# hustvl/4DGaussians

Hardware: NVIDIA H100
Metric: render FPS @300k gauss 1352x1014 (fused deform+rasterize forward); train-step ms in `train_step` (higher is better)
Workload: dtype f32

## Files before the change

### 4dgaussians_b200/csrc/g4d_api.cu

```cuda
#include <cstdio>
#include <cstdlib>
#include <atomic>
#include <cstring>
#include <mutex>
#include <string>
#include <vector>

#include "g4d_internal.h"

using namespace g4d;

namespace {

thread_local std::string t_last_error;

int fail(int code, const char* what, const char* detail = nullptr) {
    t_last_error = what;
    if (detail) { t_last_error += ": "; t_last_error += detail; }
    return code;
}

#define G4D_CUDA(expr)                                                                      \
    do {                                                                                    \
        cudaError_t e__ = (expr);                                                           \
// ... 114 lines not shown
};

namespace g4d {
int g_pdl = []() { const char* e = getenv("G4D_PDL"); return e ? atoi(e) != 0 : 1; }();
}

namespace {

struct StageTimer {
    G4DContext* c; int stage; cudaStream_t st; bool on;
    StageTimer(G4DContext* c_, int stage_, cudaStream_t st_) : c(c_), stage(stage_), st(st_), on(c_->ws->stage_timing != 0) {
        if (!on) return;
        if (!c->ev_created) {
            for (int i = 0; i < 2 * G4D_STAGE_COUNT; ++i) cudaEventCreate(&c->ev[i]);
            c->ev_created = true;
        }
        cudaEventRecord(c->ev[2 * stage], st);
    }
    ~StageTimer() {
        if (!on) return;
        cudaEventRecord(c->ev[2 * stage + 1], st);
        c->ev_used[stage] = true;
    }
};
void reset_stage_flags(G4DContext* c, int first, int last) { for (int i = first; i <= last; ++i) c->ev_used[i] = false; }

int ensure_geom(G4DContext* c, int64_t n) {
    const size_t N = (size_t)(n > 0 ? n : 1);
    GeomBuffers& g = c->g;
    auto layout = [&](Carve& m) {
        g.rec0 = m.take<float4>(N); g.rec1 = m.take<float4>(N); g.rec2 = m.take<float2>(N); g.radii = m.take<int32_t>(N);
        g.rect = m.take<uint2>(N); g.tiles_touched = m.take<uint32_t>(N); g.clamped = m.take<uint8_t>(N); g.perm = m.take<uint32_t>(N);
    };
    G4D_CUDA(ensure_layout(c->geom, layout));
    g.depth_range = &c->cam.as<CameraDev>()->depth_min;
    return G4D_OK;
}

int ensure_image(G4DContext* c, int H, int W) {
    const size_t P = (size_t)H * W;
    const int gx = (W + kTile - 1) / kTile, gy = (H + kTile - 1) / kTile;
    auto layout = [&](Carve& m) {
        c->im.final_T = m.take<float>(P); c->im.n_contrib = m.take<uint32_t>(P);
        c->b.ranges = m.take<uint2>((size_t)gx * gy);
    };
    G4D_CUDA(ensure_layout(c->img, layout));
    c->H = H; c->W = W; c->grid_x = gx; c->grid_y = gy;
    return G4D_OK;
}

int ensure_bin(G4DContext* c, int64_t r) {
    const size_t R = (size_t)(r > 0 ? r : 1);
    if ((int64_t)R <= c->capacity && c->bin.p) return G4D_OK;
    G4D_CUDA(c->bin.ensure(R * 12 + 16));
    c->capacity = (int64_t)((c->bin.cap - 16) / 12);
    c->b.kbuf = c->bin.as<uint2>();
    c->b.ids_sorted = reinterpret_cast<uint32_t*>(c->b.kbuf + c->capacity);
    return G4D_OK;
}

int ensure_fused(G4DContext* c, int64_t n, bool with_sh) {
    const size_t N = (size_t)(n > 0 ? n : 1);
    FusedOutputs& fo = c->fo;
    auto layout = [&](Carve& m) {
        fo.means3D = m.take<float>(3 * N); fo.scales = m.take<float>(3 * N); fo.rotations = m.take<float>(4 * N);
        fo.opacities = m.take<float>(N); fo.rot_norm = m.take<float>(N);
        float* shs = m.take<float>(with_sh ? 48 * N : 4);
        fo.shs = with_sh ? shs : nullptr;
    };
    G4D_CUDA(ensure_layout(c->fused, layout));
    return G4D_OK;
}

int check_params(const G4DDeformParams* p) {
    if (!p) return fail(G4D_ERR_ARG, "deform params are NULL");
    if (p->levels < 1 || p->levels > G4D_MAX_LEVELS) return fail(G4D_ERR_ARG, "levels must be in 1..4");
    if (p->channels < 4 || p->channels > 32 || (p->channels & 3)) return fail(G4D_ERR_ARG, "channels must be a multiple of 4, <= 32");
    if (p->net_width != 64 && p->net_width != 128) return fail(G4D_ERR_ARG, "net_width must be 64 or 128");
    if (p->levels * p->channels > 128) return fail(G4D_ERR_ARG, "levels*channels must be <= 128");
    for (int l = 0; l < p->levels; ++l)
        for (int a = 0; a < 4; ++a)
            if (p->res[l][a] < 2 || p->res[l][a] > 65535) return fail(G4D_ERR_ARG, "plane resolution out of range");
    return G4D_OK;
}

int refresh_packed(G4DWorkspace* ws, const G4DDeformParams* p, cudaStream_t st) {
    const size_t F = (size_t)p->levels * p->channels, WD = (size_t)p->net_width;
    auto pack = [&](void* blob, FfmaWeights* w) {
        w->w0t = static_cast<float*>(blob);
        for (int h = 0; h < G4D_NUM_HEADS; ++h) w->w1t[h] = w->w0t + F * WD + h * WD * WD;
        return launch_pack_weights(*p, w->w0t, w->w1t, st);
    };
    G4D_CUDA(ws->packed.refresh(p, 0, (F * WD + G4D_NUM_HEADS * WD * WD) * 4, pack));
    return G4D_OK;
}

int refresh_tc(G4DWorkspace* ws, const G4DDeformParams* p, cudaStream_t st) {
    const int arith = ws->tensor_cores == 2 ? 2 : 1;
    if (arith == 2 && ws->pinned->f16_range) {
        ws->pinned->f16_range = 0;
        ws->tc.valid = false;
        return fail(G4D_ERR_OVERFLOW, "an earlier FP16x2 tensor-core launch met a value outside the f16 operand range (activation >= 8188, "
                                      "feature >= 1023 or weight >= 255): its results were saturated; set G4D_OPT_TENSOR_CORES = 1 (3xTF32)");
    }
    auto pack = [&](void* blob, TcWeights* w) {
        w->arith = arith;
        w->status = &ws->pinned->f16_range;
        return launch_tc_pack_weights(*p, arith, static_cast<float*>(blob), w, st);
    };
    G4D_CUDA(ws->tc.refresh(p, arith, tc_packed_floats(*p) * 4, pack));
// ... 108 lines not shown
            const cudaError_t q = cudaEventQuery(c->ev_r[s]);
            if (q == cudaErrorNotReady) { (void)cudaGetLastError(); continue; }
            G4D_CUDA(q);
        }
        c->pending[s] = false;
        c->R = (int64_t)c->h_r[s];
        if (c->R > c->used_capacity[s]) {
            const int64_t need = c->R + c->R / 2;
            if (need > c->ws->min_capacity) c->ws->min_capacity = need;
            c->has_forward = false;
            char msg[160];
            snprintf(msg, sizeof(msg), "%lld tile instances did not fit the capacity of %lld used by an earlier no-sync forward; its image is incomplete",
                     (long long)c->R, (long long)c->used_capacity[s]);
            return fail(G4D_ERR_OVERFLOW, "instance buffer overflow", msg);
        }
    }
    return G4D_OK;
}

int bin_and_blend(G4DContext* c, const G4DCamera* cam, int64_t n, float* out_color, float* out_depth, cudaStream_t st) {
    G4DWorkspace* ws = c->ws;
    const CameraDev* dcam = c->cam.as<CameraDev>();
    int rc;
    const int num_tiles = c->grid_x * c->grid_y;
    const uint32_t kNoCap = 0xFFFFFFFFu;
    const uint32_t* readback = nullptr;
    if (n > 0) {
        if (ws->sm_count > 1024) return fail(G4D_ERR_ARG, "more than 1024 SMs are not supported by the binning kernel");
        G4D_CUDA(c->binaux.ensure(bin_aux_bytes(n, num_tiles, ws->sm_count)));
        const bool nosync = !ws->sync_mode && !(cam->debug & G4D_CAM_DEBUG) && c->capacity > 0 && c->learned;
        if (nosync && ws->min_capacity > c->capacity && (rc = ensure_bin(c, ws->min_capacity)) != G4D_OK) return rc;
        BinLayout lay{};
        {
            StageTimer tm(c, G4D_STAGE_SCAN, st);
            G4D_CUDA(launch_bin_sort(n, c->grid_x, c->grid_y, c->g, c->binaux.p, ws->tight_cull, ws->sm_count, &lay, st));
        }
        c->bin_ctl = lay.ctl;
        if (!nosync) {
            G4D_CUDA(cudaMemcpyAsync(&ws->pinned->num_rendered, &lay.ctl->R, sizeof(uint32_t), cudaMemcpyDeviceToHost, st));
            G4D_CUDA(cudaStreamSynchronize(st));
            const int64_t R = (int64_t)ws->pinned->num_rendered;
            c->R = R; c->learned = true;
            int64_t want = R;
            if (!ws->sync_mode) want = R + R / 2;
            if (want < ws->min_capacity) want = ws->min_capacity;
            if ((rc = ensure_bin(c, want)) != G4D_OK) return rc;
        } else {
            readback = &lay.ctl->R;
        }
        if ((rc = debug_sync(cam, st, "bin_sort")) != G4D_OK) return rc;
        {
            StageTimer tm(c, G4D_STAGE_EMIT, st);
            const uint32_t cap_place = (uint32_t)(c->capacity < (int64_t)kNoCap ? c->capacity : (int64_t)kNoCap);
            G4D_CUDA(launch_bin_place(c->grid_x, c->grid_y, c->g, lay, c->b.ids_sorted, c->b.kbuf, c->b.ranges, cap_place, ws->tight_cull, st));
        }
    } else {
        c->R = 0;
        G4D_CUDA(cudaMemsetAsync(c->b.ranges, 0, sizeof(uint2) * (size_t)num_tiles, st));
        if ((rc = ensure_bin(c, 1)) != G4D_OK) return rc;
    }
    if ((rc = debug_sync(cam, st, "binning")) != G4D_OK) return rc;
    {
        StageTimer tm(c, G4D_STAGE_BLEND, st);
        G4D_CUDA(launch_blend_forward(dcam, c->grid_x, c->grid_y, c->g, c->b, c->im, out_color, out_depth, ws->warp_cull, st));
    }
    if (readback) {
        const int sl = c->slot;
        c->slot = (c->slot + 1) % G4DContext::kSlots;
        G4D_CUDA(cudaMemcpyAsync(c->h_r + sl, readback, sizeof(uint32_t), cudaMemcpyDeviceToHost, st));
        G4D_CUDA(cudaEventRecord(c->ev_r[sl], st));
        c->pending[sl] = true; c->used_capacity[sl] = c->capacity;
    }
    if ((rc = debug_sync(cam, st, "blend_forward")) != G4D_OK) return rc;
    c->n = n;
    c->has_forward = true;
    return G4D_OK;
}

template <class Sh, class T> Sh caller_sh(bool split, T* dc, T* rest = nullptr) {
    return split ? Sh{nullptr, dc, rest} : Sh{dc, nullptr, nullptr};
}

int raster_backward_stages(G4DContext* c, const G4DCamera* cam, int64_t n, const RasterInputs& in, const float* dL_dcolor,
                           float* g_means3D, float* g_means2D, const ShOut& g_sh, float* g_opacities, float* g_scales,
                           float* g_rotations, cudaStream_t st) {
    const CameraDev* dcam = c->cam.as<CameraDev>();
    const size_t N = (size_t)(n > 0 ? n : 1);
    G4D_CUDA(c->gscratch.ensure(N * 8 * 4 + 256));
    float* g_mean2D = c->gscratch.as<float>();
    float* g_conic = g_mean2D + 2 * N;
    float* g_rgb = g_conic + 3 * N;
    if (n == 0) return G4D_OK;
    G4D_CUDA(cudaMemsetAsync(g_mean2D, 0, N * 8 * 4, st));
    G4D_CUDA(cudaMemsetAsync(g_opacities, 0, N * 4, st));
    reset_stage_flags(c, G4D_STAGE_BLEND_BWD, G4D_STAGE_DEFORM_BWD);
    {
        StageTimer tm(c, G4D_STAGE_BLEND_BWD, st);
        G4D_CUDA(launch_blend_backward(dcam, c->grid_x, c->grid_y, c->g, c->b, c->im, dL_dcolor, g_mean2D, g_conic, g_opacities,
                                       g_rgb, c->ws->warp_cull, st));
    }
    int rc;
    if ((rc = debug_sync(cam, st, "blend_backward")) != G4D_OK) return rc;
    StageTimer tm(c, G4D_STAGE_GEOM_BWD, st);
    G4D_CUDA(launch_preprocess_backward(dcam, n, in, c->g, g_mean2D, g_conic, g_rgb, g_means3D, g_means2D, g_scales,
                                        g_rotations, g_sh, st));
    return debug_sync(cam, st, "preprocess_backward");
}
// ... 670 lines not shown
```

### 4dgaussians_b200/csrc/g4d_bin.cu

```cuda
#include <cooperative_groups.h>
#include <cstddef>

#include "g4d_internal.h"
#include "raster_cull.cuh"

namespace cg = cooperative_groups;

namespace g4d {

namespace {

constexpr int kBinThreads = 1024;
constexpr int kDigitBits = 9;
constexpr int kRadix = 1 << kDigitBits;
constexpr uint32_t kSortSmemBytes = 32u * kRadix * 4u;

__device__ __forceinline__ uint32_t block_scan_incl(uint32_t v, uint32_t* s_w, uint32_t& total) {
    const int lane = threadIdx.x & 31, warp = threadIdx.x >> 5;
    uint32_t x = v;
#pragma unroll
    for (int o = 1; o < 32; o <<= 1) {
        const uint32_t y = __shfl_up_sync(0xffffffffu, x, o);
        if (lane >= o) x += y;
    }
// ... 27 lines not shown
            const uint32_t target = gen * G;
            uint32_t v;
            do { asm volatile("ld.acquire.gpu.global.u32 %0, [%1];" : "=r"(v) : "l"(ctr) : "memory"); } while (v < target);
        }
        __syncthreads();
    }
};

#define G4D_BIN_MARK(i) do { if (blockIdx.x == 0 && threadIdx.x == 0) a.ctl->phase_clk[i] = clock64(); } while (0)
#define G4D_BIN_MARK1(i) do { if (FIRST) G4D_BIN_MARK(i); } while (0)

struct SortShared {
    uint32_t hist[kRadix];
    uint32_t part[4 * kRadix];
    uint32_t base[kRadix];
    uint32_t sw[33];
    uint32_t mm[2];
};

template <bool FIRST, bool LAST>
__device__ __forceinline__ uint32_t radix_pass(const BinSortArgs& a, GridBar& grid, SortShared& s, uint32_t* wc, int shift,
                                               uint32_t kmin, uint32_t count, const uint32_t* __restrict__ kin,
                                               const uint32_t* __restrict__ vin, uint32_t* __restrict__ kout,
                                               uint32_t* __restrict__ vout) {
    const int tid = threadIdx.x, lane = tid & 31, warp = tid >> 5;
    const uint32_t G = gridDim.x, c = blockIdx.x;
    const uint32_t per = (count + G - 1) / G;
    const uint32_t lo = min(c * per, count), hi = min(lo + per, count);
    auto load = [&](uint32_t i, uint32_t& key, uint32_t& val) -> bool {
        if (FIRST) {
            if (a.tiles_touched[i] == 0) return false;
            key = __float_as_uint(a.rec2[i].y) - kmin;
            val = i;
            return true;
        }
        key = kin[i]; val = vin[i];
        return true;
    };
    if (tid < kRadix) s.hist[tid] = 0;
    __syncthreads();
    for (uint32_t i = lo + tid; i < hi; i += kBinThreads) {
        uint32_t key, val;
        if (load(i, key, val)) atomicAdd(&s.hist[(key >> shift) & (kRadix - 1)], 1u);
    }
    __syncthreads();
    if (tid < kRadix) a.H[c * kRadix + tid] = s.hist[tid];
    G4D_BIN_MARK1(6);
    grid.sync();
    G4D_BIN_MARK1(7);
    {
        const uint32_t d = tid & (kRadix - 1), q = tid >> kDigitBits;
        const uint32_t qs = (G + 1) / 2, c0 = q * qs, c1 = min(G, c0 + qs);
        uint32_t tot = 0, bef = 0;
        for (uint32_t cc = c0; cc < c1; ++cc) {
            const uint32_t v = __ldcg(a.H + cc * kRadix + d);
            tot += v;
            if (cc < c) bef += v;
        }
        s.part[q * kRadix + d] = tot;
        s.part[(2 + q) * kRadix + d] = bef;
    }
    __syncthreads();
    uint32_t tot = 0, bef = 0;
    if (tid < kRadix) { tot = s.part[tid] + s.part[kRadix + tid]; bef = s.part[2 * kRadix + tid] + s.part[3 * kRadix + tid]; }
    uint32_t total;
    const uint32_t incl = block_scan_incl(tot, s.sw, total);
    if (tid < kRadix) s.base[tid] = incl - tot + bef;
    __syncthreads();
    G4D_BIN_MARK1(8);
    for (uint32_t b0 = lo; b0 < hi; b0 += kBinThreads) {
        for (int j = tid; j < 32 * kRadix; j += kBinThreads) wc[j] = 0;
        __syncthreads();
        const uint32_t i = b0 + tid;
        uint32_t key = 0, val = 0;
        const bool valid = i < hi && load(i, key, val);
        const uint32_t digit = (key >> shift) & (kRadix - 1);
        const uint32_t peers = __match_any_sync(0xffffffffu, valid ? digit : ((uint32_t)kRadix + (uint32_t)lane));
        const uint32_t rank = __popc(peers & ((1u << lane) - 1u));
        if (valid && rank == 0) wc[warp * kRadix + digit] = __popc(peers);
        __syncthreads();
        if (tid < kRadix) {
            uint32_t run = s.base[tid];
#pragma unroll 8
            for (int w = 0; w < 32; ++w) {
                const uint32_t t = wc[w * kRadix + tid];
                wc[w * kRadix + tid] = run;
                run += t;
            }
            s.base[tid] = run;
        }
        __syncthreads();
        if (valid) {
            const uint32_t pos = wc[warp * kRadix + digit] + rank;
            if (!LAST) kout[pos] = key;
            vout[pos] = val;
        }
        __syncthreads();
    }
    G4D_BIN_MARK1(9);
    grid.sync();
    G4D_BIN_MARK1(10);
    return total;
}

template <class F, class F4>
__device__ __forceinline__ void walk_unordered(const uint32_t* __restrict__ perm, const uint2* __restrict__ rect,
                                               const float4* __restrict__ rec0, const float4* __restrict__ rec1, int tight, uint32_t ks,
// ... 138 lines not shown
    const uint32_t cs = __ldcg(a.chunk_start + c), ce = __ldcg(a.chunk_start + c + 1);
    {
        const uint32_t len = ce - cs, wper = (len + 31) / 32;
        const uint32_t ks = cs + min((uint32_t)warp * wper, len), ke = cs + min((uint32_t)(warp + 1) * wper, len);
        for (int y0 = 0; y0 < a.grid_y; y0 += a.count_band_rows) {
            const int y1 = min(a.grid_y, y0 + a.count_band_rows);
            const int bn = (y1 - y0) * a.grid_x;
            for (int j = tid; j < bn; j += kBinThreads) dyn[j] = 0;
            __syncthreads();
            walk_unordered(a.perm, a.rect, a.rec0, a.rec1, a.tight, ks, ke, y0, y1, a.grid_x,
                           [&](int tile, uint32_t, uint32_t) { atomicAdd(&dyn[tile], 1u); },
                           [&](const int (&tl)[4], uint32_t, uint32_t) {
#pragma unroll
                               for (int u = 0; u < 4; ++u) if (tl[u] >= 0) atomicAdd(&dyn[tl[u]], 1u);
                           });
            __syncthreads();
            for (int j = tid; j < bn; j += kBinThreads) a.M[(size_t)(y0 * a.grid_x + j) * G + c] = dyn[j];
            __syncthreads();
        }
    }
    grid.sync();

    G4D_BIN_MARK(4);
    {
        uint32_t my_total = 0;
        for (uint32_t t = c * 32u + warp; t < (uint32_t)a.num_tiles; t += G * 32u) {
            uint32_t* row = a.M + (size_t)t * G;
            uint32_t run = 0;
            for (uint32_t j0 = 0; j0 < G; j0 += 32) {
                const uint32_t j = j0 + lane;
                const uint32_t v = j < G ? __ldcg(row + j) : 0u;
                uint32_t x = v;
#pragma unroll
                for (int o = 1; o < 32; o <<= 1) {
                    const uint32_t y = __shfl_up_sync(0xffffffffu, x, o);
                    if (lane >= o) x += y;
                }
                if (j < G) row[j] = run + x - v;
                run += __shfl_sync(0xffffffffu, x, 31);
            }
            if (lane == 0) { a.tile_total[t] = run; my_total += run; }
        }
        uint32_t cta_total;
        block_scan_incl(my_total, s.sw, cta_total);
        if (tid == 0) {
            if (cta_total) atomicAdd(&a.ctl->R, cta_total);
            if (c == 0) a.ctl->n_visible = nvis;
        }
    }
    G4D_BIN_MARK(5);
    if (blockIdx.x == 0 && threadIdx.x == 0) a.ctl->phase_clk[15] = (long long)kbits;
}

__global__ void __launch_bounds__(kBinThreads, 1) bin_place_kernel(BinPlaceArgs a) {
    extern __shared__ __align__(16) uint32_t cur[];
    __shared__ uint32_t s_w[33];
    const int tid = threadIdx.x, warp = tid >> 5;
    const uint32_t c = blockIdx.x, G = gridDim.x;
    pdl_wait();
    pdl_trigger();
    const uint32_t cs = a.chunk_start[c], ce = a.chunk_start[c + 1];
    const uint32_t len = ce - cs, per = (len + 31) / 32;
    const uint32_t ks = cs + min((uint32_t)warp * per, len), ke = cs + min((uint32_t)(warp + 1) * per, len);
    for (int y0 = 0; y0 < a.grid_y; y0 += a.band_rows) {
        const int y1 = min(a.grid_y, y0 + a.band_rows);
        const uint32_t bn = (uint32_t)((y1 - y0) * a.grid_x), t0 = (uint32_t)(y0 * a.grid_x);
        {
            uint32_t before = 0;
            for (uint32_t t = tid; t < t0; t += kBinThreads) before += __ldg(a.tile_total + t);
            uint32_t run;
            block_scan_incl(before, s_w, run);
            for (uint32_t b0 = 0; b0 < bn; b0 += kBinThreads) {
                const uint32_t t = b0 + tid;
                const uint32_t v = t < bn ? __ldg(a.tile_total + t0 + t) : 0u;
                uint32_t tot;
                const uint32_t start = run + block_scan_incl(v, s_w, tot) - v;
                if (t < bn) {
                    cur[t] = start + a.M[(size_t)(t0 + t) * G + c];
                    if (c == 0) {
                        a.tile_start[t0 + t] = start;
                        a.ranges[t0 + t] = v ? make_uint2(min(start, a.capacity), min(start + v, a.capacity)) : make_uint2(0u, 0u);
                    }
                }
                run += tot;
            }
        }
        __syncthreads();
        walk_unordered(a.perm, a.rect, a.rec0, a.rec1, a.tight, ks, ke, y0, y1, a.grid_x,
                       [&](int tile, uint32_t k, uint32_t gi) {
                           const uint32_t slot = atomicAdd(&cur[tile], 1u);
                           if (slot < a.capacity) a.kbuf[slot] = make_uint2(k, gi);
                       },
                       [&](const int (&tl)[4], uint32_t k, uint32_t gi) {
                           uint32_t slot[4];
#pragma unroll
                           for (int u = 0; u < 4; ++u) slot[u] = tl[u] >= 0 ? atomicAdd(&cur[tl[u]], 1u) : 0xFFFFFFFFu;
#pragma unroll
                           for (int u = 0; u < 4; ++u) if (slot[u] < a.capacity) a.kbuf[slot[u]] = make_uint2(k, gi);
                       });
        __syncthreads();
    }
}

template <int T>
__device__ __forceinline__ void rank_tier(const BinPlaceArgs& a, uint32_t lo, uint32_t n) {
    constexpr bool kKeepId = T <= 16;
    const bool mine = n <= (uint32_t)T;
    uint32_t key[T], id[kKeepId ? T : 1];
#pragma unroll
    for (int q = 0; q < T; ++q) {
        key[q] = 0xFFFFFFFFu;
        if (mine && (uint32_t)q < n) {
            if (kKeepId) { const uint2 e = a.kbuf[lo + q]; key[q] = e.x; id[q] = e.y; }
            else key[q] = a.kbuf[lo + q].x;
        }
    }
#pragma unroll
    for (int q = 0; q < T; ++q) {
        uint32_t r = 0;
#pragma unroll
        for (int p = 0; p < T; ++p)
            if (p != q) r += key[p] < key[q] ? 1u : 0u;
        if (mine && (uint32_t)q < n) a.ids[lo + r] = kKeepId ? id[q] : a.kbuf[lo + q].y;
    }
}

template <int S>
__device__ __forceinline__ void coop_rank(const BinPlaceArgs& a, uint32_t lo, uint32_t n, int lane) {
    uint2 e[S];
    uint32_t r[S];
#pragma unroll
    for (int s = 0; s < S; ++s) {
        const uint32_t i = (uint32_t)lane + 32u * s;
        e[s] = i < n ? a.kbuf[lo + i] : make_uint2(0xFFFFFFFFu, 0u);
        r[s] = 0u;
    }
#pragma unroll
    for (int s2 = 0; s2 < S; ++s2) {
        if (32u * s2 >= n) break;
#pragma unroll 8
        for (int l = 0; l < 32; ++l) {
            const uint32_t kj = __shfl_sync(0xffffffffu, e[s2].x, l);
#pragma unroll
            for (int s = 0; s < S; ++s) r[s] += kj < e[s].x ? 1u : 0u;
        }
    }
#pragma unroll
    for (int s = 0; s < S; ++s)
        if ((uint32_t)lane + 32u * s < n) a.ids[lo + r[s]] = e[s].y;
}

__device__ __noinline__ void coop_rank_big(const BinPlaceArgs& a, uint32_t lo, uint32_t n, int lane) {
    constexpr int S = 8;
    for (uint32_t base = 0; base < n; base += 32u * S) {
        uint2 e[S];
        uint32_t r[S];
#pragma unroll
        for (int s = 0; s < S; ++s) {
            const uint32_t i = base + (uint32_t)lane + 32u * s;
            e[s] = i < n ? a.kbuf[lo + i] : make_uint2(0xFFFFFFFFu, 0u);
            r[s] = 0u;
        }
        uint32_t nxt = (uint32_t)lane < n ? a.kbuf[lo + lane].x : 0xFFFFFFFFu;
        for (uint32_t j0 = 0; j0 < n; j0 += 32u) {
            const uint32_t cur = nxt;
            const uint32_t jn = j0 + 32u + (uint32_t)lane;
            nxt = jn < n ? a.kbuf[lo + jn].x : 0xFFFFFFFFu;
#pragma unroll 8
            for (int l = 0; l < 32; ++l) {
                const uint32_t kj = __shfl_sync(0xffffffffu, cur, l);
#pragma unroll
                for (int s = 0; s < S; ++s) r[s] += kj < e[s].x ? 1u : 0u;
            }
        }
#pragma unroll
        for (int s = 0; s < S; ++s)
            if (base + (uint32_t)lane + 32u * s < n) a.ids[lo + r[s]] = e[s].y;
    }
}

__global__ void __launch_bounds__(256, 4) bin_fix_kernel(BinPlaceArgs a, int chunks) {
    const int lane = threadIdx.x & 31;
    const int rounds = (chunks + 31) / 32;
    pdl_wait();
    pdl_trigger();
    const uint32_t item = blockIdx.x * (blockDim.x >> 5) + (threadIdx.x >> 5);
    const uint32_t t = item / (uint32_t)rounds;
    if (t >= (uint32_t)a.num_tiles) return;
    const uint32_t* mrow = a.M + (size_t)t * chunks;
    {
        const int c = (int)(item - t * (uint32_t)rounds) * 32 + lane;
        const uint32_t total = __ldg(a.tile_total + t);
        const uint32_t start = __ldg(a.tile_start + t);
        const uint32_t m0 = c < chunks ? __ldg(mrow + c) : 0u;
        const uint32_t m1 = c + 1 < chunks ? __ldg(mrow + c + 1) : 0u;
        if (total == 0) return;
        uint32_t lo = 0, hi = 0;
        if (c < chunks) {
            lo = start + m0;
            hi = start + (c + 1 < chunks ? m1 : total);
            lo = min(lo, a.capacity); hi = min(hi, a.capacity);
        }
        const uint32_t n = hi - lo;
        const uint32_t nmax = __reduce_max_sync(0xffffffffu, n);
        uint32_t done_limit;
        if (nmax <= 4u) { rank_tier<4>(a, lo, n); done_limit = 4u; }
        else if (nmax <= 8u) { rank_tier<8>(a, lo, n); done_limit = 8u; }
        else if (nmax <= 12u) { rank_tier<12>(a, lo, n); done_limit = 12u; }
        else if (nmax <= 16u) { rank_tier<16>(a, lo, n); done_limit = 16u; }
        else if (nmax <= 24u) { rank_tier<24>(a, lo, n); done_limit = 24u; }
        else { rank_tier<32>(a, lo, n); done_limit = 32u; }
        uint32_t todo = __ballot_sync(0xffffffffu, n > done_limit);
        while (todo) {
            const int src = __ffs(todo) - 1;
            todo &= todo - 1;
            const uint32_t clo = __shfl_sync(0xffffffffu, lo, src), cnn = __shfl_sync(0xffffffffu, n, src);
            if (cnn <= 64u) coop_rank<2>(a, clo, cnn, lane);
            else if (cnn <= 128u) coop_rank<4>(a, clo, cnn, lane);
            else if (cnn <= 256u) coop_rank<8>(a, clo, cnn, lane);
            else coop_rank_big(a, clo, cnn, lane);
        }
    }
}

namespace {
constexpr size_t kCountSmemBudget = 160 * 1024;
constexpr size_t kPlaceSmemBudget = 96 * 1024;

void carve_bin_aux(Carve& m, int64_t n, int num_tiles, int sm_count, BinSortArgs& a, uint32_t*& tile_start) {
    const size_t N = (size_t)(n > 0 ? n : 1), G = (size_t)sm_count;
    a.kA = m.take<uint32_t>(N); a.vA = m.take<uint32_t>(N); a.kB = m.take<uint32_t>(N); a.vB = m.take<uint32_t>(N);
    a.H = m.take<uint32_t>(G * kRadix); a.S = m.take<uint32_t>(2 * G); a.chunk_start = m.take<uint32_t>(G + 1);
    a.M = m.take<uint32_t>(G * (size_t)num_tiles);
    a.tile_total = m.take<uint32_t>((size_t)num_tiles);
    tile_start = m.take<uint32_t>((size_t)num_tiles);
    a.ctl = m.take<BinCtl>(1);
}
}

size_t bin_aux_bytes(int64_t n, int num_tiles, int sm_count) {
    Carve m;
    BinSortArgs a{};
    uint32_t* tile_start;
    carve_bin_aux(m, n, num_tiles, sm_count, a, tile_start);
    return m.bytes();
}

cudaError_t launch_bin_sort(int64_t n, int grid_x, int grid_y, const GeomBuffers& g, void* aux, int tight, int sm_count,
                            BinLayout* out, cudaStream_t st) {
    const int num_tiles = grid_x * grid_y;
    BinSortArgs a{};
    a.n = n; a.rec2 = g.rec2; a.tiles_touched = g.tiles_touched; a.rect = g.rect; a.rec0 = g.rec0; a.rec1 = g.rec1;
    a.depth_range = g.depth_range;
    a.grid_bar = reinterpret_cast<uint32_t*>(reinterpret_cast<char*>(g.depth_range) - offsetof(CameraDev, depth_min) + offsetof(CameraDev, grid_bar));
    a.perm = g.perm;
    Carve m(aux);
    uint32_t* tile_start;
    carve_bin_aux(m, n, num_tiles, sm_count, a, tile_start);
    a.grid_x = grid_x; a.grid_y = grid_y; a.num_tiles = num_tiles; a.tight = tight;
    int rows = (int)(kCountSmemBudget / ((size_t)grid_x * 4));
    if (rows < 1) return cudaErrorInvalidValue;
    a.count_band_rows = rows < grid_y ? rows : grid_y;
    size_t smem = (size_t)a.count_band_rows * grid_x * 4;
    if (smem < kSortSmemBytes) smem = kSortSmemBytes;
    out->chunk_start = a.chunk_start; out->M = a.M; out->tile_total = a.tile_total; out->tile_start = tile_start; out->ctl = a.ctl;
    out->chunks = sm_count;
    cudaError_t e = cudaFuncSetAttribute(bin_sort_kernel, cudaFuncAttributeMaxDynamicSharedMemorySize, (int)smem);
    if (e != cudaSuccess) return e;
    void* args[] = {&a};
    return cudaLaunchCooperativeKernel((const void*)bin_sort_kernel, dim3((unsigned)sm_count), dim3(kBinThreads), args, smem, st);
}

cudaError_t launch_bin_place(int grid_x, int grid_y, const GeomBuffers& g, const BinLayout& lay, uint32_t* ids, uint2* kbuf,
                             uint2* ranges, uint32_t capacity, int tight, cudaStream_t st) {
    const int num_tiles = grid_x * grid_y;
    BinPlaceArgs a{};
    a.perm = g.perm; a.rect = g.rect; a.rec0 = g.rec0; a.rec1 = g.rec1; a.chunk_start = lay.chunk_start; a.M = lay.M;
    a.tile_total = lay.tile_total; a.tile_start = lay.tile_start; a.ranges = ranges; a.ids = ids; a.kbuf = kbuf;
    a.capacity = capacity; a.grid_x = grid_x; a.grid_y = grid_y; a.num_tiles = num_tiles; a.tight = tight;
    a.band_rows = (int)(kPlaceSmemBudget / (4 * (size_t)grid_x));
    if (a.band_rows < 1) return cudaErrorInvalidValue;
    if (a.band_rows > grid_y) a.band_rows = grid_y;
    const size_t smem = 4 * (size_t)a.band_rows * grid_x;
    cudaError_t e = cudaFuncSetAttribute(bin_place_kernel, cudaFuncAttributeMaxDynamicSharedMemorySize, (int)smem);
    if (e != cudaSuccess) return e;
    if ((e = launch_k(bin_place_kernel, dim3(lay.chunks), dim3(kBinThreads), smem, st, true, a)) != cudaSuccess) return e;
    const int rounds = (lay.chunks + 31) / 32;
    return launch_k(bin_fix_kernel, dim3((num_tiles * rounds + 7) / 8), dim3(256), 0, st, true, a, lay.chunks);
}

}
```

### 4dgaussians_b200/csrc/g4d_internal.h

```cpp
#pragma once
#include <cuda_runtime.h>
#include <stdint.h>

#include "deform_tile.cuh"
#include "g4d_common.cuh"

namespace g4d {

struct Carve {
    char* base;
    size_t off = 0;
    explicit Carve(void* b = nullptr) : base(static_cast<char*>(b)) {}
    template <class T> T* take(size_t count) {
        T* p = base ? reinterpret_cast<T*>(base + off) : nullptr;
        off += (count * sizeof(T) + 255) / 256 * 256;
        return p;
    }
    size_t bytes() const { return off; }
};

struct TimeRows {
    int levels = 0;
    int start[G4D_MAX_LEVELS * 3 + 1] = {};
    TimeRows(int levels_, const int32_t (*res)[4], int C) : levels(levels_) {
        for (int m = 0; m < 3 * levels; ++m) start[m + 1] = start[m] + res[m / 3][m % 3] * C;
    }
    size_t total() const { return (size_t)start[3 * levels]; }
    void place(float* base, float* (*rows)[3]) const {
        for (int m = 0; m < 3 * levels; ++m) rows[m / 3][m % 3] = base + start[m];
    }
};

struct GeomBuffers {
    float4* rec0;
    float4* rec1;
    float2* rec2;
    int32_t* radii;
    uint2* rect;
    uint32_t* tiles_touched;
    uint32_t* perm;
    uint32_t* depth_range;
    uint8_t* clamped;
};

struct BinBuffers {
    uint2* kbuf;
    uint32_t* ids_sorted;
    uint2* ranges;
};

struct BinCtl { uint32_t n_visible, R, overflow, pad; long long phase_clk[16]; };
struct BinSortArgs {
    int64_t n;
    const float2* rec2; const uint32_t* tiles_touched; const uint2* rect; const float4* rec0; const float4* rec1;
    const uint32_t* depth_range;
    uint32_t* grid_bar;
    uint32_t *kA, *vA, *kB, *vB;
    uint32_t* perm;
    uint32_t* H;
    uint32_t* S;
    uint32_t* chunk_start;
    uint32_t* M;
    uint32_t* tile_total;
    BinCtl* ctl;
    int grid_x, grid_y, num_tiles, count_band_rows;
    int tight;
};
struct BinPlaceArgs {
    const uint32_t* perm; const uint2* rect; const float4* rec0; const float4* rec1;
    const uint32_t* chunk_start; const uint32_t* M; const uint32_t* tile_total;
    uint32_t* tile_start;
    uint2* ranges;
    uint32_t* ids;
    uint2* kbuf;
    uint32_t capacity;
    int grid_x, grid_y, num_tiles, band_rows, tight;
};
struct BinLayout { uint32_t* chunk_start; uint32_t* M; uint32_t* tile_total; uint32_t* tile_start; BinCtl* ctl; int chunks; };
size_t bin_aux_bytes(int64_t n, int num_tiles, int sm_count);
cudaError_t launch_bin_sort(int64_t n, int grid_x, int grid_y, const GeomBuffers& g, void* aux, int tight, int sm_count,
                            BinLayout* out, cudaStream_t st);
cudaError_t launch_bin_place(int grid_x, int grid_y, const GeomBuffers& g, const BinLayout& lay, uint32_t* ids, uint2* kbuf,
                             uint2* ranges, uint32_t capacity, int tight, cudaStream_t st);

struct ImageBuffers {
    float* final_T;
    uint32_t* n_contrib;
};

constexpr int kShRow = 49;

struct ShIn {
    const float *shs, *dc, *rest;
    G4D_D float at(int64_t gi, int e) const {
        return shs ? __ldg(shs + gi * 48 + e) : e < 3 ? __ldg(dc + gi * 3 + e) : __ldg(rest + gi * 45 + (e - 3));
    }
    template <class F> G4D_D void with_coeffs(int64_t gi, F&& f) const {
        if (shs) f([=](int k, int ch) { return __ldg(shs + gi * 48 + 3 * k + ch); });
        else f([=](int k, int ch) { return k == 0 ? __ldg(dc + gi * 3 + ch) : __ldg(rest + gi * 45 + 3 * (k - 1) + ch); });
    }
    G4D_D void load(int64_t gi, float (&v)[48]) const {
        if (shs) {
#pragma unroll
            for (int j = 0; j < 48; j += 4) {
                const float4 b = __ldg(reinterpret_cast<const float4*>(shs + gi * 48 + j));
                v[j] = b.x; v[j + 1] = b.y; v[j + 2] = b.z; v[j + 3] = b.w;
            }
        } else {
#pragma unroll
            for (int j = 0; j < 3; ++j) v[j] = __ldg(dc + gi * 3 + j);
#pragma unroll
            for (int j = 0; j < 45; ++j) v[3 + j] = __ldg(rest + gi * 45 + j);
        }
    }
    G4D_D void stage_warp(int64_t g0, int cnt, int lane, float* rows) const {
        for (int idx = lane; idx < cnt * 48; idx += 32) {
            const int i = idx / 48, e = idx - i * 48;
            rows[i * kShRow + e] = at(g0 + i, e);
        }
    }
};

struct ShOut {
    float *shs, *dc, *rest;
    G4D_D void store_warp(int64_t g0, int cnt, int lane, const float* rows) const {
        for (int idx = lane; idx < cnt * 48; idx += 32) {
            const int i = idx / 48, e = idx - i * 48;
            const float v = rows[i * kShRow + e];
            if (shs) shs[g0 * 48 + idx] = v;
            if (e < 3) { if (dc) dc[(g0 + i) * 3 + e] = v; }
            else if (rest) rest[(g0 + i) * 45 + (e - 3)] = v;
        }
    }
};

template <class P>
// ... 129 lines not shown
```

Before: 900.9.

## Stage per-tile keys in shared memory and rank in place, dropping global kbuf

Rewrites the binning place step so each chunk stages its (key) entries per tile in shared memory and ranks them in-block before writing sorted ids directly, instead of scattering (key,id) pairs to a global kbuf and re-reading them in a separate fix kernel. Row bands are sized by actual pair counts, and bands that overflow the stage buffer fall back to a windowed pass in the fix kernel, which early-exits otherwise. The digit-histogram prefix loop is also unrolled by six. This removes a global round trip and the 12-byte-per-pair bin buffer, at the cost of much larger shared memory use and more complex overflow handling.

```diff
diff --git a/4dgaussians_b200/csrc/g4d_api.cu b/4dgaussians_b200/csrc/g4d_api.cu
--- a/4dgaussians_b200/csrc/g4d_api.cu
+++ b/4dgaussians_b200/csrc/g4d_api.cu
@@ -190,10 +190,9 @@
 int ensure_bin(G4DContext* c, int64_t r) {
     const size_t R = (size_t)(r > 0 ? r : 1);
     if ((int64_t)R <= c->capacity && c->bin.p) return G4D_OK;
-    G4D_CUDA(c->bin.ensure(R * 12 + 16));
-    c->capacity = (int64_t)((c->bin.cap - 16) / 12);
-    c->b.kbuf = c->bin.as<uint2>();
-    c->b.ids_sorted = reinterpret_cast<uint32_t*>(c->b.kbuf + c->capacity);
+    G4D_CUDA(c->bin.ensure(R * 4 + 16));
+    c->capacity = (int64_t)((c->bin.cap - 16) / 4);
+    c->b.ids_sorted = c->bin.as<uint32_t>();
     return G4D_OK;
 }
 
@@ -408,7 +407,7 @@
         {
             StageTimer tm(c, G4D_STAGE_EMIT, st);
             const uint32_t cap_place = (uint32_t)(c->capacity < (int64_t)kNoCap ? c->capacity : (int64_t)kNoCap);
-            G4D_CUDA(launch_bin_place(c->grid_x, c->grid_y, c->g, lay, c->b.ids_sorted, c->b.kbuf, c->b.ranges, cap_place, ws->tight_cull, st));
+            G4D_CUDA(launch_bin_place(c->grid_x, c->grid_y, c->g, lay, c->b.ids_sorted, c->b.ranges, cap_place, ws->tight_cull, st));
         }
     } else {
         c->R = 0;
diff --git a/4dgaussians_b200/csrc/g4d_bin.cu b/4dgaussians_b200/csrc/g4d_bin.cu
--- a/4dgaussians_b200/csrc/g4d_bin.cu
+++ b/4dgaussians_b200/csrc/g4d_bin.cu
@@ -103,7 +103,18 @@
         const uint32_t d = tid & (kRadix - 1), q = tid >> kDigitBits;
         const uint32_t qs = (G + 1) / 2, c0 = q * qs, c1 = min(G, c0 + qs);
         uint32_t tot = 0, bef = 0;
-        for (uint32_t cc = c0; cc < c1; ++cc) {
+        uint32_t cc = c0;
+        for (; cc + 6u <= c1; cc += 6u) {
+            uint32_t v[6];
+#pragma unroll
+            for (int u = 0; u < 6; ++u) v[u] = __ldcg(a.H + (cc + u) * kRadix + d);
+#pragma unroll
+            for (int u = 0; u < 6; ++u) {
+                tot += v[u];
+                if (cc + u < c) bef += v[u];
+            }
+        }
+        for (; cc < c1; ++cc) {
             const uint32_t v = __ldcg(a.H + cc * kRadix + d);
             tot += v;
             if (cc < c) bef += v;
@@ -348,197 +359,244 @@
     if (blockIdx.x == 0 && threadIdx.x == 0) a.ctl->phase_clk[15] = (long long)kbits;
 }
 
-__global__ void __launch_bounds__(kBinThreads, 1) bin_place_kernel(BinPlaceArgs a) {
-    extern __shared__ __align__(16) uint32_t cur[];
-    __shared__ uint32_t s_w[33];
-    const int tid = threadIdx.x, warp = tid >> 5;
-    const uint32_t c = blockIdx.x, G = gridDim.x;
-    pdl_wait();
-    pdl_trigger();
+namespace {
+constexpr int kLaneTier = 16;
+constexpr int kCoopBlock = 256;
+constexpr int kScanPer = 7;
+
+struct PlaceSmem {
+    uint32_t* rowcnt;
+    uint32_t* base;
+    uint32_t* cur;
+    uint32_t* items;
+    uint32_t* stage;
+};
+
+template <int T>
+__device__ __forceinline__ void lane_rank(const BinPlaceArgs& a, const uint32_t* stage, uint32_t s, uint32_t n, uint32_t dst) {
+    uint32_t key[T], r[T];
+#pragma unroll
+    for (int q = 0; q < T; ++q) key[q] = (uint32_t)q < n ? stage[s + q] : 0xFFFFFFFFu;
+#pragma unroll
+    for (int q = 0; q < T; ++q) {
+        r[q] = 0u;
+#pragma unroll
+        for (int p = 0; p < T; ++p) r[q] += key[p] < key[q] ? 1u : 0u;
+    }
+#pragma unroll
+    for (int q = 0; q < T; ++q) if ((uint32_t)q < n) key[q] = a.perm[key[q]];
+#pragma unroll
+    for (int q = 0; q < T; ++q) if ((uint32_t)q < n && dst + r[q] < a.capacity) a.ids[dst + r[q]] = key[q];
+}
+
+__device__ __forceinline__ void coop_rank_block(const BinPlaceArgs& a, const uint32_t* stage, uint32_t s, uint32_t n, uint32_t b0,
+                                                uint32_t dst, int lane) {
+    constexpr int S = kCoopBlock / 32;
+    uint32_t e[S], r[S];
+#pragma unroll
+    for (int q = 0; q < S; ++q) {
+        const uint32_t i = b0 + (uint32_t)lane + 32u * q;
+        e[q] = i < n ? stage[s + i] : 0xFFFFFFFFu;
+        r[q] = 0u;
+    }
+#pragma unroll 4
+    for (uint32_t j = 0; j < n; ++j) {
+        const uint32_t kj = stage[s + j];
+#pragma unroll
+        for (int q = 0; q < S; ++q) r[q] += kj < e[q] ? 1u : 0u;
+    }
+#pragma unroll
+    for (int q = 0; q < S; ++q) if (b0 + (uint32_t)lane + 32u * q < n) e[q] = a.perm[e[q]];
+#pragma unroll
+    for (int q = 0; q < S; ++q)
+        if (b0 + (uint32_t)lane + 32u * q < n && dst + r[q] < a.capacity) a.ids[dst + r[q]] = e[q];
+}
+
+__device__ __forceinline__ void place_band(const BinPlaceArgs& a, const PlaceSmem& sm, uint32_t* s_items, uint32_t ws, uint32_t we,
+                                        int y0, int y1, uint32_t bn) {
+    const int tid = threadIdx.x, lane = tid & 31, warp = tid >> 5;
+    if (tid == 0) *s_items = 0u;
+    const uint32_t len = we - ws, per = (len + 31) / 32;
+    const uint32_t ks = ws + min((uint32_t)warp * per, len), ke = ws + min((uint32_t)(warp + 1) * per, len);
+    __syncthreads();
+    walk_unordered(a.perm, a.rect, a.rec0, a.rec1, a.tight, ks, ke, y0, y1, a.grid_x,
+                   [&](int tile, uint32_t k, uint32_t) {
+                       const uint32_t slot = atomicAdd(&sm.cur[tile], 1u);
+                       if (slot < a.stage_cap) sm.stage[slot] = k;
+                   },
+                   [&](const int (&tl)[4], uint32_t k, uint32_t) {
+                       uint32_t slot[4];
+#pragma unroll
+                       for (int u = 0; u < 4; ++u) slot[u] = tl[u] >= 0 ? atomicAdd(&sm.cur[tl[u]], 1u) : 0xFFFFFFFFu;
+#pragma unroll
+                       for (int u = 0; u < 4; ++u) if (slot[u] < a.stage_cap) sm.stage[slot[u]] = k;
+                   });
+    __syncthreads();
+    for (uint32_t b0 = 0; b0 < bn; b0 += kBinThreads) {
+        const uint32_t t = b0 + tid;
+        uint32_t s = 0, n = 0, dst = 0;
+        if (t < bn) { s = t ? sm.cur[t - 1] : 0u; n = sm.cur[t] - s; dst = sm.base[t]; }
+        const uint32_t nl = n <= (uint32_t)kLaneTier ? n : 0u;
+        const uint32_t nmax = __reduce_max_sync(0xffffffffu, nl);
+        if (nmax > 8u) lane_rank<16>(a, sm.stage, s, nl, dst);
+        else if (nmax > 4u) lane_rank<8>(a, sm.stage, s, nl, dst);
+        else if (nmax > 0u) lane_rank<4>(a, sm.stage, s, nl, dst);
+        if (n > (uint32_t)kLaneTier) {
+            const uint32_t nb = (n + kCoopBlock - 1) / kCoopBlock, i0 = atomicAdd(s_items, nb);
+            for (uint32_t j = 0; j < nb; ++j) if (i0 + j < a.item_cap) sm.items[i0 + j] = t << 16 | j;
+        }
+    }
+    __syncthreads();
+    const uint32_t ni = min(*s_items, a.item_cap);
+    for (uint32_t i = (uint32_t)warp; i < ni; i += kBinThreads / 32) {
+        const uint32_t it = sm.items[i], t = it >> 16;
+        const uint32_t s = t ? sm.cur[t - 1] : 0u, n = sm.cur[t] - s;
+        coop_rank_block(a, sm.stage, s, n, (it & 0xFFFFu) * kCoopBlock, sm.base[t], lane);
+    }
+    __syncthreads();
+}
+}
+
+namespace {
+template <bool FIX>
+__device__ __forceinline__ void place_chunk(const BinPlaceArgs& a, uint32_t G) {
+    extern __shared__ __align__(16) uint32_t dyn[];
+    __shared__ uint32_t s_w[33], s_items;
+    PlaceSmem sm;
+    sm.rowcnt = dyn; sm.base = sm.rowcnt + a.grid_y; sm.cur = sm.base + a.table; sm.items = sm.cur + a.table;
+    sm.stage = sm.items + a.item_cap;
+    const int tid = threadIdx.x, lane = tid & 31, warp = tid >> 5;
+    const uint32_t c = blockIdx.x;
+    const uint32_t gx = (uint32_t)a.grid_x;
+    if (!FIX && tid == 0) a.fix_rows[c] = 0u;
     const uint32_t cs = a.chunk_start[c], ce = a.chunk_start[c + 1];
-    const uint32_t len = ce - cs, per = (len + 31) / 32;
-    const uint32_t ks = cs + min((uint32_t)warp * per, len), ke = cs + min((uint32_t)(warp + 1) * per, len);
-    for (int y0 = 0; y0 < a.grid_y; y0 += a.band_rows) {
-        const int y1 = min(a.grid_y, y0 + a.band_rows);
-        const uint32_t bn = (uint32_t)((y1 - y0) * a.grid_x), t0 = (uint32_t)(y0 * a.grid_x);
+    auto count = [&](uint32_t t, uint32_t& m) -> uint32_t {
+        const uint32_t* row = a.M + (size_t)t * G;
+        m = row[c];
+        return (c + 1 < G ? row[c + 1] : a.tile_total[t]) - m;
+    };
+    for (int y = warp; y < a.grid_y; y += kBinThreads / 32) {
+        uint32_t sum = 0, m;
+        for (uint32_t x = (uint32_t)lane; x < gx; x += 32) sum += count((uint32_t)y * gx + x, m);
+        sum = __reduce_add_sync(0xffffffffu, sum);
+        if (lane == 0) sm.rowcnt[y] = sum;
+    }
+    __syncthreads();
+    for (int y0 = 0; y0 < a.grid_y;) {
+        uint32_t pairs = sm.rowcnt[y0];
+        int y1 = y0 + 1;
+        const bool windowed = pairs > a.stage_cap;
+        if (!windowed)
+            while (y1 < a.grid_y && (uint32_t)(y1 + 1 - y0) * gx <= a.table && pairs + sm.rowcnt[y1] <= a.stage_cap) pairs += sm.rowcnt[y1++];
+        if (!FIX && windowed && tid == 0) a.fix_rows[c] = 1u;
+        if (FIX && !windowed) { y0 = y1; continue; }
+        const uint32_t bn = (uint32_t)(y1 - y0) * gx, t0 = (uint32_t)y0 * gx;
         {
             uint32_t before = 0;
             for (uint32_t t = tid; t < t0; t += kBinThreads) before += __ldg(a.tile_total + t);
-            uint32_t run;
+            uint32_t run, orun = 0;
             block_scan_incl(before, s_w, run);
-            for (uint32_t b0 = 0; b0 < bn; b0 += kBinThreads) {
-                const uint32_t t = b0 + tid;
-                const uint32_t v = t < bn ? __ldg(a.tile_total + t0 + t) : 0u;
-                uint32_t tot;
-                const uint32_t start = run + block_scan_incl(v, s_w, tot) - v;
-                if (t < bn) {
-                    cur[t] = start + a.M[(size_t)(t0 + t) * G + c];
-                    if (c == 0) {
-                        a.tile_start[t0 + t] = start;
-                        a.ranges[t0 + t] = v ? make_uint2(min(start, a.capacity), min(start + v, a.capacity)) : make_uint2(0u, 0u);
+            for (uint32_t b0 = 0; b0 < bn; b0 += kBinThreads * kScanPer) {
+                const uint32_t tb = b0 + (uint32_t)tid * kScanPer;
+                uint32_t v[kScanPer], m[kScanPer], cnt[kScanPer], vs = 0, cs_ = 0;
+#pragma unroll
+                for (int j = 0; j < kScanPer; ++j) {
+                    v[j] = 0u; m[j] = 0u; cnt[j] = 0u;
+                    if (tb + j < bn) { v[j] = __ldg(a.tile_total + t0 + tb + j); cnt[j] = count(t0 + tb + j, m[j]); }
+                }
+#pragma unroll
+                for (int j = 0; j < kScanPer; ++j) { vs += v[j]; cs_ += cnt[j]; }
+                uint32_t tot, ctot;
+                uint32_t start = run + block_scan_incl(vs, s_w, tot) - vs;
+                uint32_t off = orun + block_scan_incl(cs_, s_w, ctot) - cs_;
+#pragma unroll
+                for (int j = 0; j < kScanPer; ++j) {
+                    const uint32_t t = tb + j;
+                    if (t < bn) {
+                        sm.base[t] = start + m[j];
+                        sm.cur[t] = windowed ? 0u : off;
+                        if (!FIX && c == 0) {
+                            a.ranges[t0 + t] = v[j] ? make_uint2(min(start, a.capacity), min(start + v[j], a.capacity)) : make_uint2(0u, 0u);
+                        }
                     }
+                    start += v[j]; off += cnt[j];
                 }
-                run += tot;
+                run += tot; orun += ctot;
             }
         }
         __syncthreads();
-        walk_unordered(a.perm, a.rect, a.rec0, a.rec1, a.tight, ks, ke, y0, y1, a.grid_x,
-                       [&](int tile, uint32_t k, uint32_t gi) {
-                           const uint32_t slot = atomicAdd(&cur[tile], 1u);
-                           if (slot < a.capacity) a.kbuf[slot] = make_uint2(k, gi);
-                       },
-                       [&](const int (&tl)[4], uint32_t k, uint32_t gi) {
-                           uint32_t slot[4];
-#pragma unroll
-                           for (int u = 0; u < 4; ++u) slot[u] = tl[u] >= 0 ? atomicAdd(&cur[tl[u]], 1u) : 0xFFFFFFFFu;
-#pragma unroll
-                           for (int u = 0; u < 4; ++u) if (slot[u] < a.capacity) a.kbuf[slot[u]] = make_uint2(k, gi);
-                       });
-        __syncthreads();
-    }
-}
-
-template <int T>
-__device__ __forceinline__ void rank_tier(const BinPlaceArgs& a, uint32_t lo, uint32_t n) {
-    constexpr bool kKeepId = T <= 16;
-    const bool mine = n <= (uint32_t)T;
-    uint32_t key[T], id[kKeepId ? T : 1];
-#pragma unroll
-    for (int q = 0; q < T; ++q) {
-        key[q] = 0xFFFFFFFFu;
-        if (mine && (uint32_t)q < n) {
-            if (kKeepId) { const uint2 e = a.kbuf[lo + q]; key[q] = e.x; id[q] = e.y; }
-            else key[q] = a.kbuf[lo + q].x;
-        }
-    }
-#pragma unroll
-    for (int q = 0; q < T; ++q) {
-        uint32_t r = 0;
-#pragma unroll
-        for (int p = 0; p < T; ++p)
-            if (p != q) r += key[p] < key[q] ? 1u : 0u;
-        if (mine && (uint32_t)q < n) a.ids[lo + r] = kKeepId ? id[q] : a.kbuf[lo + q].y;
-    }
-}
-
-template <int S>
-__device__ __forceinline__ void coop_rank(const BinPlaceArgs& a, uint32_t lo, uint32_t n, int lane) {
-    uint2 e[S];
-    uint32_t r[S];
-#pragma unroll
-    for (int s = 0; s < S; ++s) {
-        const uint32_t i = (uint32_t)lane + 32u * s;
-        e[s] = i < n ? a.kbuf[lo + i] : make_uint2(0xFFFFFFFFu, 0u);
-        r[s] = 0u;
-    }
-#pragma unroll
-    for (int s2 = 0; s2 < S; ++s2) {
-        if (32u * s2 >= n) break;
-#pragma unroll 8
-        for (int l = 0; l < 32; ++l) {
-            const uint32_t kj = __shfl_sync(0xffffffffu, e[s2].x, l);
-#pragma unroll
-            for (int s = 0; s < S; ++s) r[s] += kj < e[s].x ? 1u : 0u;
-        }
-    }
-#pragma unroll
-    for (int s = 0; s < S; ++s)
-        if ((uint32_t)lane + 32u * s < n) a.ids[lo + r[s]] = e[s].y;
-}
-
-__device__ __noinline__ void coop_rank_big(const BinPlaceArgs& a, uint32_t lo, uint32_t n, int lane) {
-    constexpr int S = 8;
-    for (uint32_t base = 0; base < n; base += 32u * S) {
-        uint2 e[S];
-        uint32_t r[S];
-#pragma unroll
-        for (int s = 0; s < S; ++s) {
-            const uint32_t i = base + (uint32_t)lane + 32u * s;
-            e[s] = i < n ? a.kbuf[lo + i] : make_uint2(0xFFFFFFFFu, 0u);
-            r[s] = 0u;
-        }
-        uint32_t nxt = (uint32_t)lane < n ? a.kbuf[lo + lane].x : 0xFFFFFFFFu;
-        for (uint32_t j0 = 0; j0 < n; j0 += 32u) {
-            const uint32_t cur = nxt;
-            const uint32_t jn = j0 + 32u + (uint32_t)lane;
-            nxt = jn < n ? a.kbuf[lo + jn].x : 0xFFFFFFFFu;
-#pragma unroll 8
-            for (int l = 0; l < 32; ++l) {
-                const uint32_t kj = __shfl_sync(0xffffffffu, cur, l);
-#pragma unroll
-                for (int s = 0; s < S; ++s) r[s] += kj < e[s].x ? 1u : 0u;
-            }
-        }
-#pragma unroll
-        for (int s = 0; s < S; ++s)
-            if (base + (uint32_t)lane + 32u * s < n) a.ids[lo + r[s]] = e[s].y;
-    }
-}
-
-__global__ void __launch_bounds__(256, 4) bin_fix_kernel(BinPlaceArgs a, int chunks) {
-    const int lane = threadIdx.x & 31;
-    const int rounds = (chunks + 31) / 32;
+        if (!windowed) {
+            place_band(a, sm, &s_items, cs, ce, y0, y1, bn);
+        } else if (FIX) {
+            const uint32_t W = a.stage_cap / gx;
+            for (uint32_t w0 = cs; w0 < ce; w0 += W) {
+                const uint32_t w1 = min(ce, w0 + W), len = w1 - w0, per = (len + 31) / 32;
+                const uint32_t ks = w0 + min((uint32_t)warp * per, len), ke = w0 + min((uint32_t)(warp + 1) * per, len);
+                walk_unordered(a.perm, a.rect, a.rec0, a.rec1, a.tight, ks, ke, y0, y1, a.grid_x,
+                               [&](int tile, uint32_t, uint32_t) { atomicAdd(&sm.cur[tile], 1u); },
+                               [&](const int (&tl)[4], uint32_t, uint32_t) {
+#pragma unroll
+                                   for (int u = 0; u < 4; ++u) if (tl[u] >= 0) atomicAdd(&sm.cur[tl[u]], 1u);
+                               });
+                __syncthreads();
+                uint32_t orun = 0;
+                for (uint32_t b0 = 0; b0 < bn; b0 += kBinThreads) {
+                    const uint32_t t = b0 + tid;
+                    const uint32_t v = t < bn ? sm.cur[t] : 0u;
+                    uint32_t tot;
+                    const uint32_t off = orun + block_scan_incl(v, s_w, tot) - v;
+                    if (t < bn) sm.cur[t] = off;
+                    orun += tot;
+                }
+                place_band(a, sm, &s_items, w0, w1, y0, y1, bn);
+                for (uint32_t t = tid; t < bn; t += kBinThreads) {
+                    sm.base[t] += sm.cur[t] - (t ? sm.cur[t - 1] : 0u);
+                }
+                __syncthreads();
+                for (uint32_t t = tid; t < bn; t += kBinThreads) sm.cur[t] = 0u;
+                __syncthreads();
+            }
+        }
+        y0 = y1;
+    }
+}
+}
+
+__global__ void __launch_bounds__(kBinThreads, 1) bin_place_kernel(BinPlaceArgs a) {
     pdl_wait();
     pdl_trigger();
-    const uint32_t item = blockIdx.x * (blockDim.x >> 5) + (threadIdx.x >> 5);
-    const uint32_t t = item / (uint32_t)rounds;
-    if (t >= (uint32_t)a.num_tiles) return;
-    const uint32_t* mrow = a.M + (size_t)t * chunks;
-    {
-        const int c = (int)(item - t * (uint32_t)rounds) * 32 + lane;
-        const uint32_t total = __ldg(a.tile_total + t);
-        const uint32_t start = __ldg(a.tile_start + t);
-        const uint32_t m0 = c < chunks ? __ldg(mrow + c) : 0u;
-        const uint32_t m1 = c + 1 < chunks ? __ldg(mrow + c + 1) : 0u;
-        if (total == 0) return;
-        uint32_t lo = 0, hi = 0;
-        if (c < chunks) {
-            lo = start + m0;
-            hi = start + (c + 1 < chunks ? m1 : total);
-            lo = min(lo, a.capacity); hi = min(hi, a.capacity);
-        }
-        const uint32_t n = hi - lo;
-        const uint32_t nmax = __reduce_max_sync(0xffffffffu, n);
-        uint32_t done_limit;
-        if (nmax <= 4u) { rank_tier<4>(a, lo, n); done_limit = 4u; }
-        else if (nmax <= 8u) { rank_tier<8>(a, lo, n); done_limit = 8u; }
-        else if (nmax <= 12u) { rank_tier<12>(a, lo, n); done_limit = 12u; }
-        else if (nmax <= 16u) { rank_tier<16>(a, lo, n); done_limit = 16u; }
-        else if (nmax <= 24u) { rank_tier<24>(a, lo, n); done_limit = 24u; }
-        else { rank_tier<32>(a, lo, n); done_limit = 32u; }
-        uint32_t todo = __ballot_sync(0xffffffffu, n > done_limit);
-        while (todo) {
-            const int src = __ffs(todo) - 1;
-            todo &= todo - 1;
-            const uint32_t clo = __shfl_sync(0xffffffffu, lo, src), cnn = __shfl_sync(0xffffffffu, n, src);
-            if (cnn <= 64u) coop_rank<2>(a, clo, cnn, lane);
-            else if (cnn <= 128u) coop_rank<4>(a, clo, cnn, lane);
-            else if (cnn <= 256u) coop_rank<8>(a, clo, cnn, lane);
-            else coop_rank_big(a, clo, cnn, lane);
-        }
-    }
-}
+    place_chunk<false>(a, gridDim.x);
+}
+
+__global__ void __launch_bounds__(kBinThreads, 1) bin_fix_kernel(BinPlaceArgs a, int chunks) {
+    pdl_wait();
+    pdl_trigger();
+    if (a.fix_rows[blockIdx.x] == 0u) return;
+    place_chunk<true>(a, (uint32_t)chunks);
+}
+
 
 namespace {
 constexpr size_t kCountSmemBudget = 160 * 1024;
-constexpr size_t kPlaceSmemBudget = 96 * 1024;
-
-void carve_bin_aux(Carve& m, int64_t n, int num_tiles, int sm_count, BinSortArgs& a, uint32_t*& tile_start) {
+constexpr size_t kPlaceSmemBytes = 220 * 1024;
+constexpr uint32_t kPlaceTableMax = 6400;
+
+void carve_bin_aux(Carve& m, int64_t n, int num_tiles, int sm_count, BinSortArgs& a, uint32_t*& fix_rows) {
     const size_t N = (size_t)(n > 0 ? n : 1), G = (size_t)sm_count;
     a.kA = m.take<uint32_t>(N); a.vA = m.take<uint32_t>(N); a.kB = m.take<uint32_t>(N); a.vB = m.take<uint32_t>(N);
     a.H = m.take<uint32_t>(G * kRadix); a.S = m.take<uint32_t>(2 * G); a.chunk_start = m.take<uint32_t>(G + 1);
     a.M = m.take<uint32_t>(G * (size_t)num_tiles);
     a.tile_total = m.take<uint32_t>((size_t)num_tiles);
-    tile_start = m.take<uint32_t>((size_t)num_tiles);
     a.ctl = m.take<BinCtl>(1);
+    fix_rows = m.take<uint32_t>(G);
 }
 }
 
 size_t bin_aux_bytes(int64_t n, int num_tiles, int sm_count) {
     Carve m;
     BinSortArgs a{};
-    uint32_t* tile_start;
-    carve_bin_aux(m, n, num_tiles, sm_count, a, tile_start);
+    uint32_t* fix_rows;
+    carve_bin_aux(m, n, num_tiles, sm_count, a, fix_rows);
     return m.bytes();
 }
 
@@ -551,15 +609,16 @@
     a.grid_bar = reinterpret_cast<uint32_t*>(reinterpret_cast<char*>(g.depth_range) - offsetof(CameraDev, depth_min) + offsetof(CameraDev, grid_bar));
     a.perm = g.perm;
     Carve m(aux);
-    uint32_t* tile_start;
-    carve_bin_aux(m, n, num_tiles, sm_count, a, tile_start);
+    uint32_t* fix_rows;
+    carve_bin_aux(m, n, num_tiles, sm_count, a, fix_rows);
     a.grid_x = grid_x; a.grid_y = grid_y; a.num_tiles = num_tiles; a.tight = tight;
     int rows = (int)(kCountSmemBudget / ((size_t)grid_x * 4));
     if (rows < 1) return cudaErrorInvalidValue;
     a.count_band_rows = rows < grid_y ? rows : grid_y;
     size_t smem = (size_t)a.count_band_rows * grid_x * 4;
     if (smem < kSortSmemBytes) smem = kSortSmemBytes;
-    out->chunk_start = a.chunk_start; out->M = a.M; out->tile_total = a.tile_total; out->tile_start = tile_start; out->ctl = a.ctl;
+    out->chunk_start = a.chunk_start; out->M = a.M; out->tile_total = a.tile_total; out->ctl = a.ctl;
+    out->fix_rows = fix_rows;
     out->chunks = sm_count;
     cudaError_t e = cudaFuncSetAttribute(bin_sort_kernel, cudaFuncAttributeMaxDynamicSharedMemorySize, (int)smem);
     if (e != cudaSuccess) return e;
@@ -567,22 +626,25 @@
     return cudaLaunchCooperativeKernel((const void*)bin_sort_kernel, dim3((unsigned)sm_count), dim3(kBinThreads), args, smem, st);
 }
 
-cudaError_t launch_bin_place(int grid_x, int grid_y, const GeomBuffers& g, const BinLayout& lay, uint32_t* ids, uint2* kbuf,
-                             uint2* ranges, uint32_t capacity, int tight, cudaStream_t st) {
-    const int num_tiles = grid_x * grid_y;
+cudaError_t launch_bin_place(int grid_x, int grid_y, const GeomBuffers& g, const BinLayout& lay, uint32_t* ids, uint2* ranges,
+                             uint32_t capacity, int tight, cudaStream_t st) {
+    const uint32_t num_tiles = (uint32_t)grid_x * (uint32_t)grid_y;
     BinPlaceArgs a{};
     a.perm = g.perm; a.rect = g.rect; a.rec0 = g.rec0; a.rec1 = g.rec1; a.chunk_start = lay.chunk_start; a.M = lay.M;
-    a.tile_total = lay.tile_total; a.tile_start = lay.tile_start; a.ranges = ranges; a.ids = ids; a.kbuf = kbuf;
-    a.capacity = capacity; a.grid_x = grid_x; a.grid_y = grid_y; a.num_tiles = num_tiles; a.tight = tight;
-    a.band_rows = (int)(kPlaceSmemBudget / (4 * (size_t)grid_x));
-    if (a.band_rows < 1) return cudaErrorInvalidValue;
-    if (a.band_rows > grid_y) a.band_rows = grid_y;
-    const size_t smem = 4 * (size_t)a.band_rows * grid_x;
-    cudaError_t e = cudaFuncSetAttribute(bin_place_kernel, cudaFuncAttributeMaxDynamicSharedMemorySize, (int)smem);
+    a.tile_total = lay.tile_total; a.ranges = ranges; a.ids = ids; a.fix_rows = lay.fix_rows;
+    a.capacity = capacity; a.grid_x = grid_x; a.grid_y = grid_y; a.num_tiles = (int)num_tiles; a.tight = tight;
+    a.table = num_tiles < kPlaceTableMax ? num_tiles : kPlaceTableMax;
+    if (a.table < (uint32_t)grid_x) a.table = (uint32_t)grid_x;
+    const int64_t words = (int64_t)(kPlaceSmemBytes / 4) - grid_y - 2 * (int64_t)a.table;
+    if (a.table >= 65536u || words < 17) return cudaErrorInvalidValue;
+    a.stage_cap = (uint32_t)((words - 1) * kLaneTier / (kLaneTier + 1));
+    a.item_cap = (uint32_t)words - a.stage_cap;
+    if (a.stage_cap < (uint32_t)grid_x) return cudaErrorInvalidValue;
+    cudaError_t e = cudaFuncSetAttribute(bin_place_kernel, cudaFuncAttributeMaxDynamicSharedMemorySize, (int)kPlaceSmemBytes);
     if (e != cudaSuccess) return e;
-    if ((e = launch_k(bin_place_kernel, dim3(lay.chunks), dim3(kBinThreads), smem, st, true, a)) != cudaSuccess) return e;
-    const int rounds = (lay.chunks + 31) / 32;
-    return launch_k(bin_fix_kernel, dim3((num_tiles * rounds + 7) / 8), dim3(256), 0, st, true, a, lay.chunks);
-}
-
-}
+    if ((e = cudaFuncSetAttribute(bin_fix_kernel, cudaFuncAttributeMaxDynamicSharedMemorySize, (int)kPlaceSmemBytes)) != cudaSuccess) return e;
+    if ((e = launch_k(bin_place_kernel, dim3(lay.chunks), dim3(kBinThreads), kPlaceSmemBytes, st, true, a)) != cudaSuccess) return e;
+    return launch_k(bin_fix_kernel, dim3(lay.chunks), dim3(kBinThreads), kPlaceSmemBytes, st, true, a, lay.chunks);
+}
+
+}
diff --git a/4dgaussians_b200/csrc/g4d_internal.h b/4dgaussians_b200/csrc/g4d_internal.h
--- a/4dgaussians_b200/csrc/g4d_internal.h
+++ b/4dgaussians_b200/csrc/g4d_internal.h
@@ -44,7 +44,6 @@
 };
 
 struct BinBuffers {
-    uint2* kbuf;
     uint32_t* ids_sorted;
     uint2* ranges;
 };
@@ -69,19 +68,19 @@
 struct BinPlaceArgs {
     const uint32_t* perm; const uint2* rect; const float4* rec0; const float4* rec1;
     const uint32_t* chunk_start; const uint32_t* M; const uint32_t* tile_total;
-    uint32_t* tile_start;
     uint2* ranges;
     uint32_t* ids;
-    uint2* kbuf;
+    uint32_t* fix_rows;
     uint32_t capacity;
-    int grid_x, grid_y, num_tiles, band_rows, tight;
-};
-struct BinLayout { uint32_t* chunk_start; uint32_t* M; uint32_t* tile_total; uint32_t* tile_start; BinCtl* ctl; int chunks; };
+    int grid_x, grid_y, num_tiles, tight;
+    uint32_t table, item_cap, stage_cap;
+};
+struct BinLayout { uint32_t* chunk_start; uint32_t* M; uint32_t* tile_total; BinCtl* ctl; uint32_t* fix_rows; int chunks; };
 size_t bin_aux_bytes(int64_t n, int num_tiles, int sm_count);
 cudaError_t launch_bin_sort(int64_t n, int grid_x, int grid_y, const GeomBuffers& g, void* aux, int tight, int sm_count,
                             BinLayout* out, cudaStream_t st);
-cudaError_t launch_bin_place(int grid_x, int grid_y, const GeomBuffers& g, const BinLayout& lay, uint32_t* ids, uint2* kbuf,
-                             uint2* ranges, uint32_t capacity, int tight, cudaStream_t st);
+cudaError_t launch_bin_place(int grid_x, int grid_y, const GeomBuffers& g, const BinLayout& lay, uint32_t* ids, uint2* ranges,
+                             uint32_t capacity, int tight, cudaStream_t st);
 
 struct ImageBuffers {
     float* final_T;
```

After: 947.2 (median of 6 runs). 1.05x the previous value.
